# jianzongwu/betrayed-by-captions

Hardware: AMD Instinct MI355X
Metric: images/sec (COCO-shaped 1024x1024, 100 queries, forward-only) (higher is better)
Workload: dtype f32; 1 GPU; configs[1]: R50 + 100 queries, 1024x1024, batch 2/GPU, forward-only; global_batch=2, parallelism=replicas x1, precision=fp32 (parity mode, f16x3 MFMA), hip_graph=True, x3_overflow=False, library_fallbacks=0

## Files before the change

betrayed-by-captions_amd/_lib.py:

```python
import ctypes
import os

import torch

_HERE = os.path.dirname(os.path.abspath(__file__))
LIB_PATH = os.path.join(_HERE, 'lib', 'libcgg_hip.so')

CGG_F32 = 0
CGG_BF16 = 1

_c_int = ctypes.c_int
_c_vp = ctypes.c_void_p
_c_f = ctypes.c_float
_c_i64 = ctypes.c_int64

PROTOTYPES = {
    'cgg_version': (_c_int, []),
    'cgg_init': (_c_int, [_c_int]),
    'cgg_msda_forward_fused_vld': (_c_int, [_c_vp, _c_int, _c_vp, _c_vp, _c_vp, _c_int, _c_vp, _c_vp] + [_c_int] * 7 + [_c_vp]),
    'cgg_msda_backward_hostlevels_ws': (_c_int, [_c_vp, _c_int] + [_c_vp] * 8 + [_c_int] * 8 + [_c_vp, _c_i64, _c_vp, _c_vp]),
    'cgg_msda_backward_workspace_bytes': (_c_i64, [_c_vp, _c_vp] + [_c_int] * 7),
    'cgg_msda_read_levels': (_c_int, [_c_vp, _c_vp, _c_int, _c_int, _c_vp, _c_vp, _c_vp]),
    'cgg_last_error_string': (ctypes.c_char_p, []),
    'cgg_msda_forward': (_c_int, [_c_vp] * 6 + [_c_int] * 8 + [_c_vp]),
# ... 7 lines not shown
    'cgg_mask_logits': (_c_int, [_c_vp] * 5 + [_c_int] * 4 + [_c_vp]),
    'cgg_mask_logits_bits_astat': (_c_int, [_c_vp] * 3 + [_c_int] * 4 + [_c_vp]),
    'cgg_mask_logits_f32': (_c_int, [_c_vp] * 4 + [_c_int] * 4 + [_c_vp]),
    'cgg_mask_logits_backward_workspace_bytes': (_c_i64, [_c_int] * 4),
    'cgg_mask_logits_backward': (_c_int, [_c_vp] * 6 + [_c_int] * 5 + [_c_vp]),
    'cgg_attn_mask_fix_full_rows': (_c_int, [_c_vp, _c_int, _c_int, _c_vp]),
    'cgg_attn_mask_from_logits': (_c_int, [_c_vp, _c_vp] + [_c_int] * 5 + [_c_vp]),
    'cgg_masked_xattn_workspace_bytes': (_c_i64, [_c_int] * 5),
    'cgg_masked_xattn_forward': (_c_int, [_c_vp] * 5 + [_c_int] * 5 + [_c_f, _c_int, _c_vp]),
    'cgg_masked_xattn_forward_strided': (_c_int, [_c_vp, _c_vp, _c_int, _c_i64, _c_vp, _c_vp, _c_vp] + [_c_int] * 5 + [_c_f, _c_vp]),
    'cgg_masked_xattn_forward_x3': (_c_int, [_c_vp, _c_vp, _c_int, _c_i64, _c_vp, _c_vp, _c_vp] + [_c_int] * 5 + [_c_f, _c_vp]),
    'cgg_masked_xattn_forward_lse': (_c_int, [_c_vp] * 6 + [_c_int] * 5 + [_c_f, _c_int, _c_vp]),
    'cgg_masked_xattn_backward_workspace_bytes': (_c_i64, [_c_int] * 5),
    'cgg_masked_xattn_backward': (_c_int, [_c_vp] * 9 + [_c_int] * 5 + [_c_f, _c_int, _c_vp]),
    'cgg_masked_xattn_backward_x3': (_c_int, [_c_vp] * 10 + [_c_int] * 5 + [_c_f, _c_vp]),
    'cgg_window_attn_forward': (_c_int, [_c_vp] * 4 + [_c_int] * 7 + [_c_f, _c_vp]),
    'cgg_window_attn_backward_workspace_bytes': (_c_i64, [_c_int] * 5),
    'cgg_window_attn_backward': (_c_int, [_c_vp] * 7 + [_c_int] * 7 + [_c_f, _c_vp]),
    'cgg_grounding_pair_costs': (_c_int, [_c_vp] * 4 + [_c_int] * 5 + [_c_f, _c_vp]),
    'cgg_grounding_pair_costs_backward': (_c_int, [_c_vp] * 5 + [_c_int] * 5 + [_c_f, _c_vp]),
    'cgg_ce_rows_forward': (_c_int, [_c_vp] * 4 + [_c_int, _c_int, _c_i64, _c_i64, _c_int, _c_vp]),
    'cgg_ce_rows_backward': (_c_int, [_c_vp] * 4 + [_c_int, _c_int, _c_i64, _c_i64, _c_int, _c_vp]),
    'cgg_match_cost_rows': (_c_int, [_c_vp] * 4 + [_c_int, _c_int, _c_int, _c_vp]),
    'cgg_rle_encode_bitmasks': (_c_i64, [_c_vp, _c_int, _c_int, _c_int, _c_i64, _c_int, _c_int, _c_vp, _c_i64, _c_vp]),
    'cgg_masked_xattn_forward_bf16': (_c_int, [_c_vp] * 6 + [_c_int] * 5 + [_c_f, _c_int, _c_i64, _c_int, _c_vp]),
    'cgg_linear_rows': (_c_int, [_c_vp, _c_int, _c_vp, _c_vp, _c_vp, _c_int, _c_vp] + [_c_int] * 6 + [_c_vp]),
    'cgg_add_layernorm': (_c_int, [_c_vp] * 5 + [_c_int, _c_int, _c_f, _c_vp]),
    'cgg_linear_rows_packed_bytes': (_c_i64, [_c_int, _c_int]),
    'cgg_linear_rows_pack': (_c_int, [_c_vp, _c_vp, _c_int, _c_int, _c_vp]),
    'cgg_linear_rows_bf16': (_c_int, [_c_vp, _c_int, _c_vp, _c_vp, _c_vp, _c_int, _c_vp, _c_int, _c_vp, _c_vp, _c_f,
                                      _c_vp, _c_int, _c_vp, _c_int] + [_c_int] * 5 +
                             [_c_vp, _c_int, _c_int, _c_vp, _c_int, _c_int, _c_vp]),
    'cgg_decoder_tail_bf16': (_c_int, [_c_vp, _c_int, _c_i64, _c_int, _c_vp, _c_vp, _c_f, _c_vp, _c_int, _c_vp, _c_vp, _c_f] +
                              [_c_vp] * 12 + [_c_int, _c_int, _c_vp]),
    'cgg_self_attn_rows_bf16': (_c_int, [_c_vp, _c_int, _c_vp, _c_int, _c_vp] + [_c_int] * 4 + [_c_f, _c_vp]),
    'cgg_decoder_mid_bf16': (_c_int, [_c_vp, _c_int, _c_vp, _c_vp, _c_vp, _c_int, _c_vp, _c_vp, _c_f, _c_vp, _c_int] +
                             [_c_vp] * 5 + [_c_int, _c_int, _c_vp]),
    'cgg_decoder_ffn_bf16': (_c_int, [_c_vp, _c_int] + [_c_vp] * 5 + [_c_int] * 3 + [_c_vp]),
    'cgg_x3_packed_bytes': (_c_i64, [_c_int, _c_int]),
    'cgg_x3_pack': (_c_int, [_c_vp, _c_vp, _c_int, _c_int, _c_vp]),
    'cgg_linear_rows_x3': (_c_int, [_c_vp, _c_int, _c_vp, _c_vp, _c_vp, _c_int, _c_vp, _c_int, _c_vp, _c_vp, _c_f,
                                    _c_vp, _c_int, _c_vp, _c_int] + [_c_int] * 5 +
                           [_c_vp, _c_int, _c_int, _c_vp, _c_int, _c_int, _c_vp]),
    'cgg_decoder_tail_x3': (_c_int, [_c_vp, _c_int, _c_i64, _c_int, _c_vp, _c_vp, _c_f, _c_vp, _c_int, _c_vp, _c_vp, _c_f] +
                            [_c_vp] * 12 + [_c_int, _c_int, _c_vp]),
    'cgg_decoder_mid_x3': (_c_int, [_c_vp, _c_int, _c_vp, _c_vp, _c_vp, _c_int, _c_vp, _c_vp, _c_f, _c_vp, _c_int] +
                           [_c_vp] * 5 + [_c_int, _c_int, _c_vp]),
    'cgg_decoder_ffn_x3': (_c_int, [_c_vp, _c_int] + [_c_vp] * 5 + [_c_int] * 3 + [_c_vp]),
    'cgg_encoder_layer_tail_x3': (_c_int, [_c_vp] * 6 + [_c_f] + [_c_vp] * 6 + [_c_f, _c_vp, _c_int, _c_vp, _c_vp] +
                                  [_c_int] * 3 + [_c_vp]),
    'cgg_gemm_x3': (_c_int, [_c_vp, _c_int, _c_vp, _c_vp, _c_vp, _c_int, _c_vp, _c_int] + [_c_int] * 4 + [_c_vp]),
    'cgg_stem_conv7x7_x3_nchw': (_c_int, [_c_vp] * 4 + [_c_int] * 3 + [_c_vp]),
    'cgg_bias_relu_maxpool_nhwc_f32': (_c_int, [_c_vp] * 3 + [_c_int] * 4 + [_c_vp]),
    'cgg_gemm_x3_ex': (_c_int, [_c_vp, _c_int, _c_vp, _c_vp, _c_vp, _c_int, _c_int, _c_vp, _c_int, _c_vp, _c_int, _c_int] +
                       [_c_int] * 4 + [_c_vp]),
    'cgg_conv_x3_nhwc': (_c_int, [_c_vp] * 5 + [_c_int] * 10 + [_c_vp]),
    'cgg_gemm_x3s': (_c_int, [_c_vp, _c_int, _c_vp, _c_vp, _c_vp, _c_int, _c_int, _c_int, _c_vp, _c_int, _c_int] + [_c_int] * 4 + [_c_vp]),
    'cgg_gemm_x3s_batched': (_c_int, [_c_vp, _c_int, _c_int, _c_i64, _c_vp, _c_vp, _c_vp, _c_int, _c_int, _c_int, _c_vp, _c_int, _c_int] + [_c_int] * 4 + [_c_vp]),
    'cgg_conv_x3s_nhwc': (_c_int, [_c_vp] * 4 + [_c_int, _c_vp, _c_int] + [_c_int] * 10 + [_c_vp]),
    'cgg_x3a_encode': (_c_int, [_c_vp, _c_vp, _c_i64, _c_vp]),
    'cgg_x3a_decode': (_c_int, [_c_vp, _c_vp, _c_i64, _c_vp]),
    'cgg_x3_overflow_check': (_c_int, [_c_int, _c_vp, _c_vp]),
    'cgg_gemm_x3s_cfg': (_c_int, [_c_vp, _c_int, _c_vp, _c_vp, _c_vp, _c_int, _c_int, _c_int, _c_vp, _c_int, _c_int] + [_c_int] * 5 + [_c_vp]),
    'cgg_conv_x3s_nhwc_cfg': (_c_int, [_c_vp] * 4 + [_c_int, _c_vp, _c_int] + [_c_int] * 11 + [_c_vp]),
    'cgg_bias_relu_maxpool_nhwc_f32_x3a': (_c_int, [_c_vp] * 3 + [_c_int] * 4 + [_c_vp]),
    'cgg_group_norm_nhwc_f32_x3a': (_c_int, [_c_vp] * 4 + [_c_int] * 4 + [_c_f, _c_int, _c_vp, _c_int, _c_int, _c_i64, _c_int, _c_vp,
                                             _c_i64, _c_vp, _c_vp, _c_vp]),
    'cgg_encoder_layer_tail_x3a': (_c_int, [_c_vp] * 6 + [_c_f] + [_c_vp] * 6 + [_c_f, _c_vp, _c_int, _c_vp, _c_vp] +
                                   [_c_int] * 3 + [_c_vp]),
    'cgg_group_norm_nhwc_f32_stats': (_c_int, [_c_vp, _c_vp] + [_c_int] * 4 + [_c_vp]),
    'cgg_mask_feature_head_x3': (_c_int, [_c_vp] * 4 + [_c_f, _c_int] + [_c_vp] * 5 + [_c_int, _c_vp] + [_c_int] * 5 + [_c_vp]),
    'cgg_mask_feature_head_x3_cfg': (_c_int, [_c_vp] * 4 + [_c_f, _c_int] + [_c_vp] * 5 + [_c_int, _c_vp] + [_c_int] * 6 + [_c_vp]),
    'cgg_image_prep_u8': (_c_int, [_c_vp, _c_i64, _c_i64, _c_vp, _c_int, _c_vp, _c_vp, _c_vp, _c_int, _c_int, _c_vp, _c_int, _c_int, _c_vp]),
    'cgg_wgrad_x3_workspace_bytes': (_c_i64, [_c_int] * 3),
    'cgg_wgrad_x3': (_c_int, [_c_vp, _c_int, _c_vp, _c_int, _c_vp, _c_vp] + [_c_int] * 3 + [_c_vp]),
    'cgg_wgrad_bias_x3': (_c_int, [_c_vp, _c_int, _c_vp, _c_int, _c_vp, _c_vp, _c_vp] + [_c_int] * 3 + [_c_vp]),
    'cgg_transpose_f32': (_c_int, [_c_vp, _c_vp, _c_int, _c_int, _c_int, _c_vp]),
    'cgg_nchw_to_nhwc_pad1_f32': (_c_int, [_c_vp, _c_vp] + [_c_int] * 4 + [_c_vp]),
    'cgg_topk_select': (_c_int, [_c_vp, _c_int, _c_int, _c_int, _c_int, _c_vp, _c_vp]),
    'cgg_absmax_f32': (_c_int, [_c_vp, _c_int, _c_int, _c_int, _c_vp, _c_vp]),
    'cgg_relu_bwd_absmax_f32': (_c_int, [_c_vp, _c_vp, _c_vp, ctypes.c_longlong, _c_vp, _c_vp]),
    'cgg_gemm_x3_bwd': (_c_int, [_c_vp, _c_int, _c_vp, _c_vp, _c_vp, _c_int, _c_vp, _c_int, _c_vp] + [_c_int] * 3 + [_c_vp]),
    'cgg_gemm_x3_scaled': (_c_int, [_c_vp, _c_int, _c_vp, _c_vp, _c_vp, _c_vp, _c_int, _c_vp, _c_int] + [_c_int] * 4 + [_c_vp]),
    'cgg_conv_x3_nhwc_scaled': (_c_int, [_c_vp] * 6 + [_c_int] * 10 + [_c_vp]),
    'cgg_wgrad_x3_scaled': (_c_int, [_c_vp, _c_int, _c_vp, _c_vp, _c_int, _c_vp, _c_vp, _c_vp] + [_c_int] * 3 + [_c_vp]),
    'cgg_layernorm_chain': (_c_int, [_c_vp, _c_int, _c_vp, _c_vp, _c_f, _c_vp, _c_int, _c_vp, _c_vp, _c_f, _c_vp, _c_vp,
                                     _c_vp, _c_int, _c_int, _c_int, _c_i64, _c_vp]),
    'cgg_msda_prologue': (_c_int, [_c_vp, _c_int, _c_vp, _c_vp, _c_vp, _c_vp] + [_c_int] * 5 + [_c_vp]),
    'cgg_msda_prologue_backward': (_c_int, [_c_vp, _c_vp, _c_vp, _c_int, _c_vp, _c_vp] + [_c_int] * 5 + [_c_vp]),
    'cgg_msda_forward_fused_bf16': (_c_int, [_c_vp] * 4 + [_c_int] + [_c_vp] * 2 + [_c_int] * 7 + [_c_vp]),
    'cgg_msda_forward_fused_bf16_hm': (_c_int, [_c_vp] * 4 + [_c_int] + [_c_vp] * 2 + [_c_int] * 7 + [_c_vp]),
    'cgg_decoder_kv_pack_k': (_c_int, [_c_vp, _c_vp, _c_int, _c_int, _c_vp]),
    'cgg_decoder_kv_proj_bf16': (_c_int, [_c_vp] * 7 + [_c_int] * 4 + [_c_vp]),
    'cgg_add_layernorm_backward_partials': (ctypes.c_int64, [_c_int]),
    'cgg_add_layernorm_backward': (_c_int, [_c_vp] * 5 + [_c_int, _c_vp, _c_f] + [_c_vp] * 3 + [_c_int, _c_int, _c_vp]),
    'cgg_add_layernorm_backward_amax': (_c_int, [_c_vp] * 5 + [_c_int, _c_vp, _c_f] + [_c_vp] * 4 + [_c_int, _c_int, _c_vp]),
    'cgg_bottleneck64_bf16': (_c_int, [_c_vp] * 8 + [_c_int] * 5 + [_c_vp]),
    'cgg_encoder_proj_pack': (_c_int, [_c_vp, _c_vp, _c_int, _c_int, _c_vp]),
    'cgg_encoder_proj_bf16': (_c_int, [_c_vp] * 3 + [_c_int] + [_c_vp] * 6 + [_c_int] * 5 + [_c_vp]),
    'cgg_encoder_ffn_ln_kv_bf16': (_c_int, [_c_vp] * 7 + [_c_f, _c_vp, _c_vp, _c_int, _c_vp, _c_int] + [_c_vp] * 3 +
                                   [_c_int] * 3 + [_c_vp]),
    'cgg_encoder_layer_tail_bf16': (_c_int, [_c_vp] * 6 + [_c_f] + [_c_vp] * 6 + [_c_f, _c_vp, _c_int, _c_vp, _c_vp, _c_int] +
                                    [_c_vp] * 3 + [_c_int] * 3 + [_c_vp]),
    'cgg_encoder_ffn_ln_bf16': (_c_int, [_c_vp] * 7 + [_c_f, _c_vp, _c_int] + [_c_vp] * 3 + [_c_int] * 3 + [_c_vp]),
    'cgg_add_layernorm_kv': (_c_int, [_c_vp, _c_int, _c_vp, _c_int] + [_c_vp] * 4 + [_c_int, _c_vp, _c_int] + [_c_vp] * 3 +
                             [_c_int, _c_int, _c_f, _c_vp]),
# ... 97 lines not shown
```

betrayed-by-captions_amd/backbones.py:

```python
import os

import torch
import torch.nn as nn

from . import ops, runtime
from .registry import BACKBONES

FROZEN_FOLDED = os.environ.get('CGG_FROZEN_FOLDED', '1') != '0'
X3_STEM = os.environ.get('CGG_X3_STEM', '1') != '0'


class Bottleneck(nn.Module):
    expansion = 4

    def __init__(self, inplanes, planes, stride=1, downsample=None, style='pytorch'):
        super().__init__()
        s1, s2 = (1, stride) if style == 'pytorch' else (stride, 1)
        self.conv1 = nn.Conv2d(inplanes, planes, 1, stride=s1, bias=False)
        self.bn1 = nn.BatchNorm2d(planes)
        self.conv2 = nn.Conv2d(planes, planes, 3, stride=s2, padding=1, bias=False)
        self.bn2 = nn.BatchNorm2d(planes)
        self.conv3 = nn.Conv2d(planes, planes * 4, 1, bias=False)
        self.bn3 = nn.BatchNorm2d(planes * 4)
        self.relu = nn.ReLU(inplace=True)
# ... 248 lines not shown
            if name == 'stem':
                return [fold(self.conv1, self.bn1, stem=True)]
            seq = []
            for blk in getattr(self, name):
                if blk.downsample is not None:
                    seq.append(fold(blk.downsample[0], blk.downsample[1]))
                seq.append(fold(blk.conv1, blk.bn1))
                seq.append(fold(blk.conv2, blk.bn2))
                if isinstance(blk, Bottleneck):
                    seq.append(fold(blk.conv3, blk.bn3))
            return seq

        cache = self.__dict__.setdefault('_fold_cache_x3', {})
        names = ['stem'] + list(self.res_layers if upto is None else self.res_layers[:upto])
        out = []
        for name in names:
            mods = [self.conv1, self.bn1] if name == 'stem' else [getattr(self, name)]
            tensors = [t for m in mods for t in list(m.parameters()) + list(m.buffers())]
            key = (sum(t._version for t in tensors), str(self.conv1.weight.device))
            hit = cache.get(name)
            if hit is None or hit[0] != key:
                with torch.no_grad():
                    hit = (key, stage_seq(name))
                cache[name] = hit
            out.extend(hit[1])
        return out

    def _x3_ok(self):
        def conv_ok(c):
            return (c.groups == 1 and tuple(c.dilation) == (1, 1) and c.kernel_size[0] == c.kernel_size[1]
                    and c.stride[0] == c.stride[1] and c.padding[0] == c.padding[1] and c.in_channels % 32 == 0 and c.bias is None
                    and c.out_channels % 8 == 0 and c.kernel_size[0] * c.kernel_size[1] <= 32)
        for name in self.res_layers:
            for blk in getattr(self, name):
                convs = [blk.conv1, blk.conv2] + ([blk.conv3] if isinstance(blk, Bottleneck) else [])
                if blk.downsample is not None:
                    if not (isinstance(blk.downsample[0], nn.Conv2d) and isinstance(blk.downsample[1], nn.BatchNorm2d)):
                        return False
                    convs.append(blk.downsample[0])
                if not all(conv_ok(c) for c in convs):
                    return False
        return self.conv1.bias is None

    def _forward_x3(self, x, upto=None):
        import torch.nn.functional as F
        x3a = runtime.x3a_enabled()
        seq = iter(self._folded_x3(upto))
        w, b = next(seq)
        mp, c1 = self.maxpool, self.conv1
        if ((mp.kernel_size, mp.stride, mp.padding, mp.dilation, mp.ceil_mode) == (3, 2, 1, 1, False) and x.dtype == torch.float32
                and x.is_contiguous() and tuple(c1.weight.shape) == (64, 3, 7, 7) and tuple(c1.stride) == (2, 2)
                and tuple(c1.padding) == (3, 3) and tuple(c1.dilation) == (1, 1) and X3_STEM):
            pk, sc = runtime.derived_cached('stem_packed_x3', (w,), lambda: ops.pack_stem_weight_x3(w))
            x = ops.bias_relu_maxpool_nhwc_f32(ops.stem_conv7x7_x3(x, pk, sc), b, x3a=x3a)
        else:
            x = F.conv2d(x.float(), w, b, stride=c1.stride, padding=c1.padding)
            x = mp(torch.relu_(x)).permute(0, 2, 3, 1).contiguous()
            if x3a:
                x = ops.x3a_encode(x)

        def conv(x, c, relu, res=None):
            wk, bias = next(seq)
            if x3a:
                return ops.conv_x3s_nhwc(x, wk, c.out_channels, c.kernel_size[0], c.stride[0], c.padding[0], bias, res=res, relu=relu)
            return ops.conv_x3_nhwc(x, wk, c.out_channels, c.kernel_size[0], c.stride[0], c.padding[0], bias, res=res, relu=relu)

        outs = []
        for i, name in enumerate(self.res_layers):
            if upto is not None and i >= upto:
                break
            for blk in getattr(self, name):
                identity = x if blk.downsample is None else conv(x, blk.downsample[0], False)
                y = conv(x, blk.conv1, True)
                if isinstance(blk, Bottleneck):
                    y = conv(y, blk.conv2, True)
                    x = conv(y, blk.conv3, True, identity)
                else:
                    x = conv(y, blk.conv2, True, identity)
            if i in self.out_indices:
                outs.append(x)
        if upto is not None:
            dec = (lambda t: ops.x3a_decode(t)) if x3a else (lambda t: t)
            return [dec(o) for o in outs], dec(x)
        if x3a and self.x3a_outputs:
            return tuple(ops.as_x3a(o.permute(0, 3, 1, 2)) for o in outs)
        if x3a:
            return tuple(ops.x3a_decode(o).permute(0, 3, 1, 2) for o in outs)
        return tuple(o.permute(0, 3, 1, 2) for o in outs)

    def forward(self, x):
        frozen_bn = all(not m.training for m in self.modules() if isinstance(m, nn.BatchNorm2d))
        if runtime.is_bf16() and not torch.is_grad_enabled() and frozen_bn and x.is_cuda:
            return self._forward_folded(x)
        if runtime.x3_enabled() and not torch.is_grad_enabled() and frozen_bn and x.is_cuda:
            if self._x3_ok():
                return self._forward_x3(x)
            runtime.note_fallback('ResNet', 'a convolution outside the implicit-GEMM rules (groups, dilation, C % 32, N % 8): MIOpen f32')
        outs = []
        frozen_nhwc = []
        first = 0
        xn = None
        if (FROZEN_FOLDED and runtime.x3_enabled() and torch.is_grad_enabled() and frozen_bn and x.is_cuda and self.frozen_stages >= 1
                and not x.requires_grad and self._x3_ok() and x.dtype == torch.float32
                and not any(p.requires_grad for n in self.res_layers[:self.frozen_stages] for p in getattr(self, n).parameters())
                and not any(p.requires_grad for p in list(self.conv1.parameters()) + list(self.bn1.parameters()))):
            with torch.no_grad():
                fouts, xf = self._forward_x3(x, upto=self.frozen_stages)
# ... 49 lines not shown
```

betrayed-by-captions_amd/ops.py:

```python
import ctypes
import os
import math

import torch

from . import _lib
from ._lib import CGG_BF16, CGG_F32, CggError, check, dev_ptr, stream_ptr

_WS_CACHE = {}

KERNEL_EVENTS = None


KERNEL_META = None


class _timed:
    def __init__(self, name, **meta):
        self.name = name
        self.meta = meta
        self.on = KERNEL_EVENTS is not None and not torch.cuda.is_current_stream_capturing()

    def __enter__(self):
        if self.on:
# ... 2038 lines not shown

def pack_stem_weight(w):
    if tuple(w.shape) != (64, 3, 7, 7):
        raise CggError(f'pack_stem_weight: expected (64, 3, 7, 7), got {tuple(w.shape)}')
    wk = torch.zeros((64, 7, 8, 3), dtype=torch.float32, device=w.device)
    wk[:, :, :7, :] = w.detach().float().permute(0, 2, 3, 1)
    wk = torch.cat([wk.reshape(64, 168), torch.zeros((64, 8), dtype=torch.float32, device=w.device)], 1)
    frag = wk.view(2, 32, 11, 2, 8).permute(0, 2, 3, 1, 4).contiguous().to(torch.bfloat16)
    out = frag.view(torch.uint8).reshape(-1)
    assert out.numel() == _lib_().cgg_stem_conv7x7_packed_bytes()
    return out


def stem_conv7x7(img, packed):
    B, C, H, W = img.shape
    if C != 3 or img.dtype != torch.float32 or not img.is_contiguous():
        raise CggError('stem_conv7x7: img must be a contiguous (B, 3, H, W) float32 tensor')
    Ho, Wo = (H - 1) // 2 + 1, (W - 1) // 2 + 1
    y = torch.empty((B, Ho, Wo, 64), dtype=torch.bfloat16, device=img.device)
    check(_lib_().cgg_stem_conv7x7_nchw(dev_ptr(img), dev_ptr(packed), dev_ptr(y), B, H, W, stream_ptr(img.device)),
          'cgg_stem_conv7x7_nchw')
    return y


def pack_stem_weight_x3(w):
    if tuple(w.shape) != (64, 3, 7, 7):
        raise CggError(f'pack_stem_weight_x3: expected (64, 3, 7, 7), got {tuple(w.shape)}')
    wk = torch.zeros((64, 7, 8, 3), dtype=torch.float32, device=w.device)
    wk[:, :, :7, :] = w.detach().float().permute(0, 2, 3, 1)
    wk = torch.cat([wk.reshape(64, 168), torch.zeros((64, 8), dtype=torch.float32, device=w.device)], 1)
    amax = wk.abs().amax(1).clamp_min(1e-30)
    e = torch.floor(torch.log2(amax)) + 1
    s = torch.pow(2.0, 11 - e)
    ws = wk * s[:, None]
    hi = ws.to(torch.float16)
    lo = (ws - hi.float()).to(torch.float16)
    frag = lambda t: t.view(2, 32, 11, 2, 8).permute(0, 2, 3, 1, 4).contiguous().view(torch.uint8).reshape(-1)
    packed = torch.cat([frag(hi), frag(lo)])
    assert packed.numel() == 2 * _lib_().cgg_stem_conv7x7_packed_bytes()
    return packed, (1.0 / (s * 16.0)).float().contiguous()


def stem_conv7x7_x3(img, packed, wscale):
    B, C, H, W = img.shape
    if C != 3 or img.dtype != torch.float32 or not img.is_contiguous():
        raise CggError('stem_conv7x7_x3: img must be a contiguous (B, 3, H, W) float32 tensor')
    Ho, Wo = (H - 1) // 2 + 1, (W - 1) // 2 + 1
    y = torch.empty((B, Ho, Wo, 64), dtype=torch.float32, device=img.device)
    check(_lib_().cgg_stem_conv7x7_x3_nchw(dev_ptr(img), dev_ptr(packed), dev_ptr(wscale, 'wscale', torch.float32), dev_ptr(y), B, H, W,
                                           stream_ptr(img.device)), 'cgg_stem_conv7x7_x3_nchw')
    return y


def bias_relu_maxpool_nhwc_f32(x, bias, x3a=False):
    B, H, W, C = x.shape
    Ho, Wo = (H - 1) // 2 + 1, (W - 1) // 2 + 1
    y = torch.empty((B, Ho, Wo, C), dtype=torch.float32, device=x.device)
    fn = _lib_().cgg_bias_relu_maxpool_nhwc_f32_x3a if x3a else _lib_().cgg_bias_relu_maxpool_nhwc_f32
    rc = fn(dev_ptr(x, 'x', torch.float32), dev_ptr(bias, 'bias', torch.float32), dev_ptr(y), B, H, W, C, stream_ptr(x.device))
    check(rc, 'cgg_bias_relu_maxpool_nhwc_f32')
    return y


def linear_sum_assignment_batch(costs):
    if not costs:
        return []
    flat = torch.cat([c.detach().to(device='cpu', dtype=torch.float32).contiguous().reshape(-1) for c in costs]) \
        if len(costs) > 1 else costs[0].detach().to(device='cpu', dtype=torch.float32).contiguous().reshape(-1)
    nr = [int(c.shape[0]) for c in costs]
    nc = [int(c.shape[1]) for c in costs]
    sizes = [min(a, b) for a, b in zip(nr, nc)]
    total = sum(sizes)
    rows = torch.empty((max(total, 1),), dtype=torch.int64)
    cols = torch.empty((max(total, 1),), dtype=torch.int64)
    rc = _lib_().cgg_linear_sum_assignment_f32(ctypes.c_void_p(flat.data_ptr()) if flat.numel() else None, len(costs),
                                               _int_array(nr), _int_array(nc), ctypes.c_void_p(rows.data_ptr()),
                                               ctypes.c_void_p(cols.data_ptr()))
    check(rc, 'cgg_linear_sum_assignment_f32')
    out, o = [], 0
    for n in sizes:
        out.append((rows[o:o + n], cols[o:o + n]))
        o += n
    return out


def point_sample_planes(planes, index, points):
    N, H, W = planes.shape
    rows, P, _ = points.shape
    out = torch.empty((rows, P), dtype=torch.float32, device=planes.device)
    if rows == 0:
        return out
    check(_lib_().cgg_point_sample_planes(dev_ptr(planes, 'planes', torch.float32), dev_ptr(index, 'index', torch.int32),
                                          dev_ptr(points.contiguous(), 'points', torch.float32), dev_ptr(out), N, H, W, rows, P,
                                          stream_ptr(planes.device)), 'cgg_point_sample_planes')
    return out


class _PointSampleRowsFn(torch.autograd.Function):

    @staticmethod
    def forward(ctx, planes, points):
        planes = planes.contiguous()
        points = points.contiguous()
        rows, H, W = planes.shape
        idx = torch.arange(rows, dtype=torch.int32, device=planes.device)
        ctx.save_for_backward(points)
# ... 141 lines not shown
```

include/cgg_hip.h:

```cpp
#ifndef CGG_HIP_H_
#define CGG_HIP_H_

#include <stdint.h>

#ifdef __cplusplus
extern "C" {
#endif

#define CGG_VERSION 100

#define CGG_OK 0
#define CGG_EINVAL (-1)
#define CGG_EUNSUPPORTED (-2)
#define CGG_EALIGN (-3)
#define CGG_ELIBRARY (-4)

#define CGG_F32 0
#define CGG_BF16 1
#define CGG_F32_BF16MFMA 2
#define CGG_F32_X3 3

typedef void* cgg_stream_t;

int cgg_version(void);
// ... 146 lines not shown
                        float* y, float* yp, float* z, int rows, int N, int nsum, int64_t plane,
                        cgg_stream_t stream);

int cgg_decoder_tail_bf16(const float* planes, int nsum, int64_t plane_stride, int ld, const float* gamma_a,
                          const float* beta_a, float eps_a, const float* pos, int pos_rows, const float* gamma_b,
                          const float* beta_b, float eps_b, const void* w1, const float* b1, const void* w2,
                          const float* b2, const void* w3, const float* b3, const void* wq, const float* bq, float* y,
                          float* yp, float* mask_embed, float* qn, int M, int C, cgg_stream_t stream);

int cgg_decoder_mid_bf16(const float* core, int ldc, const void* wo, const float* bo, const float* res, int ldr,
                         const float* gamma, const float* beta, float eps, const float* pos, int pos_rows,
                         const void* wqkv, const float* bqkv, float* x1, float* q, float* kv, int M, int C,
                         cgg_stream_t stream);

int cgg_decoder_ffn_bf16(const float* x, int ldx, const void* w1, const float* b1, const void* w2, const float* b2,
                         float* planes, int M, int C, int F, cgg_stream_t stream);

int64_t cgg_x3_packed_bytes(int N, int K);
int cgg_x3_pack(const float* w, void* packed, int N, int K, cgg_stream_t stream);
int cgg_linear_rows_x3(const float* x, int ldx, const void* w_x3, const float* bias, const float* res,
                       int ldr, float* y, int ldy, const float* ln_gamma, const float* ln_beta, float ln_eps,
                       const float* pos, int pos_rows, float* yp, int ldyp, int M, int N, int K, int relu_cols,
                       int ksplit, const float* x2, int ldx2, int x2_col, float* y2, int ldy2, int y2_col,
                       cgg_stream_t stream);
int cgg_decoder_tail_x3(const float* planes, int nsum, int64_t plane_stride, int ld, const float* gamma_a,
                        const float* beta_a, float eps_a, const float* pos, int pos_rows, const float* gamma_b,
                        const float* beta_b, float eps_b, const void* w1, const float* b1, const void* w2,
                        const float* b2, const void* w3, const float* b3, const void* wq, const float* bq, float* y,
                        float* yp, float* mask_embed, float* qn, int M, int C, cgg_stream_t stream);
int cgg_decoder_mid_x3(const float* core, int ldc, const void* wo, const float* bo, const float* res, int ldr,
                       const float* gamma, const float* beta, float eps, const float* pos, int pos_rows,
                       const void* wqkv, const float* bqkv, float* x1, float* q, float* kv, int M, int C,
                       cgg_stream_t stream);
int cgg_decoder_ffn_x3(const float* x, int ldx, const void* w1, const float* b1, const void* w2, const float* b2,
                       float* planes, int M, int C, int F, cgg_stream_t stream);

int cgg_group_norm_nhwc_f32(const float* x, const float* gamma, const float* beta, void* ws, int B, int HW, int C, int groups,
                            float eps, int relu, const float* up_src, int up_h, int up_w, int64_t up_bstride, int W,
                            float* y32, int64_t y32_bstride, void* y16, const float* pos, void* yp16, int64_t y16_bstride,
                            cgg_stream_t stream);
int cgg_pack_mask_feature_nhwc_f32_x3(const float* feat, void* const* hi_host, void* const* lo_host, const int* pools_host,
                                      int n, int B, int C, int H, int W, cgg_stream_t stream);
int cgg_point_sample_nhwc_x3(const float* feat, const float* pts, void* hi, void* lo, int B, int H, int W, int C, int P_total,
                             int P_group, cgg_stream_t stream);
int cgg_encoder_layer_tail_x3(const float* a32, const float* x32, const void* wo_x3, const float* bo, const float* gamma0,
                              const float* beta0, float eps0, const void* w1_x3, const float* b1, const void* w2_x3,
                              const float* b2, const float* gamma1, const float* beta1, float eps1, const float* pos,
                              int pos_rows, float* y32, float* yp32, int M, int C, int F, cgg_stream_t stream);
int cgg_gemm_x3(const float* a, int lda, const void* w_x3, const float* bias, const float* res, int ldr, float* out, int ldc,
                int M, int N, int K, int relu, cgg_stream_t stream);
int cgg_stem_conv7x7_x3_nchw(const float* img, const void* w_packed, const float* wscale, float* out, int B, int H, int W,
                             cgg_stream_t stream);
int cgg_bias_relu_maxpool_nhwc_f32(const float* x, const float* bias, float* y, int B, int H, int W, int C, cgg_stream_t stream);
int cgg_gemm_x3_ex(const float* a, int lda, const void* w_x3, const float* bias, const float* res, int ldr, int res_mod, float* out,
                   int ldc, float* out2, int ldc2, int col2, int M, int N, int K, int relu, cgg_stream_t stream);
int cgg_conv_x3_nhwc(const float* x, const void* w_x3, const float* bias, const float* res, float* out, int B, int H, int W,
                     int C, int N, int KH, int KW, int stride, int pad, int relu, cgg_stream_t stream);

int cgg_gemm_x3s(const void* a_x3a, int lda, const void* w_x3, const float* bias, const void* res, int ldr, int res_fmt,
                 int res_mod, void* out, int ldc, int out_fmt, int M, int N, int K, int relu, cgg_stream_t stream);
int cgg_gemm_x3s_batched(const void* a_x3a, int lda, int rows_per_image, int64_t a_bstride, const void* w_x3, const float* bias,
                         const void* res, int ldr, int res_fmt, int res_mod, void* out, int ldc, int out_fmt, int M, int N, int K,
                         int relu, cgg_stream_t stream);
int cgg_conv_x3s_nhwc(const void* x_x3a, const void* w_x3, const float* bias, const void* res, int res_fmt, void* out,
                      int out_fmt, int B, int H, int W, int C, int N, int KH, int KW, int stride, int pad, int relu,
                      cgg_stream_t stream);
int cgg_x3a_encode(const float* x, void* out_x3a, int64_t n, cgg_stream_t stream);
int cgg_x3a_decode(const void* x_x3a, float* out, int64_t n, cgg_stream_t stream);
int cgg_x3_overflow_check(int reset, int* value_host, cgg_stream_t stream);
int cgg_gemm_x3s_cfg(const void* a_x3a, int lda, const void* w_x3, const float* bias, const void* res, int ldr, int res_fmt,
                     int res_mod, void* out, int ldc, int out_fmt, int M, int N, int K, int relu, int cfg, cgg_stream_t stream);
int cgg_conv_x3s_nhwc_cfg(const void* x_x3a, const void* w_x3, const float* bias, const void* res, int res_fmt, void* out,
                          int out_fmt, int B, int H, int W, int C, int N, int KH, int KW, int stride, int pad, int relu, int cfg,
                          cgg_stream_t stream);
int cgg_bias_relu_maxpool_nhwc_f32_x3a(const float* x, const float* bias, void* y_x3a, int B, int H, int W, int C,
                                       cgg_stream_t stream);
int cgg_group_norm_nhwc_f32_x3a(const float* x, const float* gamma, const float* beta, void* ws, int B, int HW, int C, int groups,
                                float eps, int relu, const void* up_src_x3a, int up_h, int up_w, int64_t up_bstride, int W,
                                void* y_x3a, int64_t y_bstride, const float* pos, void* yp_x3a, cgg_stream_t stream);

int64_t cgg_group_norm_nhwc_backward_workspace_bytes(int B, int HW, int groups);
int cgg_group_norm_nhwc_f32_backward(const float* x, const float* y, const float* dy, const float* stats, const float* gamma, void* ws,
                                     int B, int HW, int C, int groups, float eps, int relu, float* dx, float* tot, float* dlo, int lo_h,
                                     int lo_w, int W, int dx_padded, cgg_stream_t stream);
int cgg_group_norm_nhwc_f32_padout(const float* x, const float* gamma, const float* beta, void* ws, int B, int HW, int C, int groups,
                                   float eps, int relu, const float* up_src, int up_h, int up_w, int64_t up_bstride, int W,
                                   float* y_padded, cgg_stream_t stream);
int cgg_encoder_layer_tail_x3a(const float* a32, const void* x_x3a, const void* wo_x3, const float* bo, const float* gamma0,
                               const float* beta0, float eps0, const void* w1_x3, const float* b1, const void* w2_x3,
                               const float* b2, const float* gamma1, const float* beta1, float eps1, const float* pos,
                               int pos_rows, void* y_x3a, void* yp_x3a, int M, int C, int F, cgg_stream_t stream);
int cgg_group_norm_nhwc_f32_stats(const float* x, void* ws, int B, int HW, int C, int groups, cgg_stream_t stream);
int cgg_mask_feature_head_x3(const float* z, const void* gn_ws, const float* gamma, const float* beta, float eps, int groups,
                             const void* w_x3, const float* bias, void* const* hi_host, void* const* lo_host, const int* pools_host,
                             int n, float* mf, int B, int H, int W, int C, int N, cgg_stream_t stream);
int cgg_mask_feature_head_x3_cfg(const float* z, const void* gn_ws, const float* gamma, const float* beta, float eps, int groups,
                                 const void* w_x3, const float* bias, void* const* hi_host, void* const* lo_host,
                                 const int* pools_host, int n, float* mf, int B, int H, int W, int C, int N, int cfg,
                                 cgg_stream_t stream);

#define CGG_IMAGE_PREP_MAX_DIM 65535
int cgg_image_prep_u8(const uint8_t* staged, int64_t staged_bytes, int64_t table_offset, const int32_t* table_host, int B,
                      const float* mean, const float* std, const float* pad_val, int to_rgb, int pad_before_norm, float* out, int Hb,
                      int Wb, cgg_stream_t stream);

int cgg_transpose_f32(const float* in, float* out, int B, int R, int C, cgg_stream_t stream);
// ... 138 lines not shown
```

Before: 396.6 images/sec.

## Fuse stem 7x7 conv with bias, ReLU and maxpool into one kernel

Adds a HIP kernel that computes the 7x7 stride-2 stem convolution with split-precision MFMA on a tile covering a 4x16 pooled output region, stages the conv results in LDS, then applies the 3x3 stride-2 maxpool, bias and ReLU, and writes the pooled NHWC output (optionally in x3a encoding with an overflow flag). This avoids writing the full-resolution conv map to global memory and reading it back in a second kernel. In exchange it recomputes the conv at pooled-tile halo borders and adds LDS pressure. The old two-kernel path stays as a fallback.

```diff
diff --git a/betrayed-by-captions_amd/_lib.py b/betrayed-by-captions_amd/_lib.py
--- a/betrayed-by-captions_amd/_lib.py
+++ b/betrayed-by-captions_amd/_lib.py
@@ -83,6 +83,7 @@
     'cgg_gemm_x3': (_c_int, [_c_vp, _c_int, _c_vp, _c_vp, _c_vp, _c_int, _c_vp, _c_int] + [_c_int] * 4 + [_c_vp]),
     'cgg_stem_conv7x7_x3_nchw': (_c_int, [_c_vp] * 4 + [_c_int] * 3 + [_c_vp]),
     'cgg_bias_relu_maxpool_nhwc_f32': (_c_int, [_c_vp] * 3 + [_c_int] * 4 + [_c_vp]),
+    'cgg_stem_pool_x3': (_c_int, [_c_vp] * 5 + [_c_int] * 4 + [_c_vp]),
     'cgg_gemm_x3_ex': (_c_int, [_c_vp, _c_int, _c_vp, _c_vp, _c_vp, _c_int, _c_int, _c_vp, _c_int, _c_vp, _c_int, _c_int] +
                        [_c_int] * 4 + [_c_vp]),
     'cgg_conv_x3_nhwc': (_c_int, [_c_vp] * 5 + [_c_int] * 10 + [_c_vp]),
diff --git a/betrayed-by-captions_amd/backbones.py b/betrayed-by-captions_amd/backbones.py
--- a/betrayed-by-captions_amd/backbones.py
+++ b/betrayed-by-captions_amd/backbones.py
@@ -324,7 +324,10 @@
                 and x.is_contiguous() and tuple(c1.weight.shape) == (64, 3, 7, 7) and tuple(c1.stride) == (2, 2)
                 and tuple(c1.padding) == (3, 3) and tuple(c1.dilation) == (1, 1) and X3_STEM):
             pk, sc = runtime.derived_cached('stem_packed_x3', (w,), lambda: ops.pack_stem_weight_x3(w))
-            x = ops.bias_relu_maxpool_nhwc_f32(ops.stem_conv7x7_x3(x, pk, sc), b, x3a=x3a)
+            if ops.stem_pool_x3_ok(x, pk, sc, b, x3a):
+                x = ops.stem_pool_x3(x, pk, sc, b, x3a=x3a)
+            else:
+                x = ops.bias_relu_maxpool_nhwc_f32(ops.stem_conv7x7_x3(x, pk, sc), b, x3a=x3a)
         else:
             x = F.conv2d(x.float(), w, b, stride=c1.stride, padding=c1.padding)
             x = mp(torch.relu_(x)).permute(0, 2, 3, 1).contiguous()
diff --git a/betrayed-by-captions_amd/csrc/stem_pool.hip b/betrayed-by-captions_amd/csrc/stem_pool.hip
--- /dev/null
+++ b/betrayed-by-captions_amd/csrc/stem_pool.hip
@@ -0,0 +1,192 @@
+#include "x3.h"
+
+typedef __attribute__((ext_vector_type(4))) uint32_t u32x4;
+
+#define SP_PH 4
+#define SP_PW 16
+#define SP_CH (2 * SP_PH + 1)
+#define SP_CW (2 * SP_PW + 1)
+#define SP_NPIX (SP_CH * SP_CW)
+#define SP_NT 10
+#define SP_THREADS (32 * SP_NT)
+#define SP_IH (2 * SP_CH + 5)
+#define SP_IWP 72
+#define SP_KS 11
+#define SP_OS 36
+
+__global__ __launch_bounds__(SP_THREADS) void cgg_stem_pool_x3_kernel(const float* __restrict__ img, const u32x4* __restrict__ wp,
+                                                                      const float* __restrict__ wscale, const float* __restrict__ bias,
+                                                                      float* __restrict__ out, int H, int W, int Ho, int Wo, int Hp,
+                                                                      int Wp, int x3a, int* __restrict__ flag) {
+  constexpr int WFRAG = 2 * SP_KS * 64;
+  constexpr int TILE_EL = SP_IH * SP_IWP * 3;
+  constexpr int LDS_MAIN = 2 * (WFRAG * 16 + TILE_EL * 2), LDS_STAGE = SP_NPIX * SP_OS * 4;
+  constexpr int LDS_BYTES = LDS_MAIN > LDS_STAGE ? LDS_MAIN : LDS_STAGE;
+  static_assert(LDS_BYTES <= 65536, "static LDS");
+  __shared__ __attribute__((aligned(16))) unsigned char lds_raw[LDS_BYTES];
+  u32x4* wl = reinterpret_cast<u32x4*>(lds_raw);
+  uint16_t* tile = reinterpret_cast<uint16_t*>(lds_raw + 2 * WFRAG * 16);
+  float* ob = reinterpret_cast<float*>(lds_raw);
+  const int tid = threadIdx.x, lane = tid & 63, wave = tid >> 6;
+  const int j = lane & 31, hi = lane >> 5;
+  const int b = blockIdx.z, py0 = blockIdx.y * SP_PH, px0 = blockIdx.x * SP_PW;
+  const int cy0 = 2 * py0 - 1, cx0 = 2 * px0 - 1;
+  const int iy0 = 2 * cy0 - 3, ix0 = 2 * cx0 - 3;
+
+  constexpr int WIT = (2 * WFRAG + SP_THREADS - 1) / SP_THREADS;
+  u32x4 wv[WIT];
+#pragma unroll
+  for (int it = 0; it < WIT; ++it) {
+    const int i = tid + SP_THREADS * it;
+    wv[it] = i < 2 * WFRAG ? wp[i] : u32x4{0u, 0u, 0u, 0u};
+  }
+
+  const float* ib = img + (size_t)b * 3 * H * W;
+  constexpr int NIT = (TILE_EL + SP_THREADS - 1) / SP_THREADS;
+  float tv[NIT];
+#pragma unroll
+  for (int it = 0; it < NIT; ++it) {
+    const int i = tid + SP_THREADS * it;
+    const int c = i / (SP_IH * SP_IWP);
+    const int rem = i - c * (SP_IH * SP_IWP);
+    const int r = rem / SP_IWP, col = rem - r * SP_IWP;
+    const int iy = iy0 + r, ix = ix0 + col;
+    tv[it] = 0.f;
+    if (i < TILE_EL && iy >= 0 && iy < H && ix >= 0 && ix < W) tv[it] = ib[((size_t)c * H + iy) * W + ix];
+  }
+#pragma unroll
+  for (int it = 0; it < NIT; ++it) {
+    const int i = tid + SP_THREADS * it;
+    const int c = i / (SP_IH * SP_IWP);
+    const int rem = i - c * (SP_IH * SP_IWP);
+    if (i < TILE_EL) {
+      uint16_t h, l;
+      cgg_x3_split1(tv[it], h, l);
+      tile[rem * 3 + c] = h;
+      tile[TILE_EL + rem * 3 + c] = l;
+    }
+  }
+#pragma unroll
+  for (int it = 0; it < WIT; ++it) {
+    const int i = tid + SP_THREADS * it;
+    if (i < 2 * WFRAG) wl[i] = wv[it];
+  }
+  __syncthreads();
+
+  int poff[2];
+#pragma unroll
+  for (int nt = 0; nt < 2; ++nt) {
+    int p = (2 * wave + nt) * 32 + j;
+    p = p < SP_NPIX ? p : SP_NPIX - 1;
+    const int r = p / SP_CW, c = p - r * SP_CW;
+    poff[nt] = (2 * r * SP_IWP + 2 * c) * 3;
+  }
+  f32x16 acc[2][2];
+#pragma unroll
+  for (int nt = 0; nt < 2; ++nt)
+#pragma unroll
+    for (int mt = 0; mt < 2; ++mt)
+#pragma unroll
+      for (int r = 0; r < 16; ++r) acc[nt][mt][r] = 0.f;
+#pragma unroll
+  for (int ks = 0; ks < SP_KS; ++ks) {
+    const int g = 2 * ks + hi;
+    const int ky = g / 3, part = g - 3 * ky;
+    const int koff = (ky > 6 ? 6 : ky) * SP_IWP * 3 + 8 * part;
+#pragma unroll
+    for (int nt = 0; nt < 2; ++nt) {
+      const uint16_t* src = tile + poff[nt] + koff;
+      const uint32_t* s32 = reinterpret_cast<const uint32_t*>(src);
+      const u32x4 bv = {s32[0], s32[1], s32[2], s32[3]};
+      const uint32_t* l32 = reinterpret_cast<const uint32_t*>(src + TILE_EL);
+      const u32x4 bl = {l32[0], l32[1], l32[2], l32[3]};
+#pragma unroll
+      for (int mt = 0; mt < 2; ++mt)
+        cgg_x3_mfma(acc[nt][mt], wl[(mt * SP_KS + ks) * 64 + lane], wl[WFRAG + (mt * SP_KS + ks) * 64 + lane], bv, bl);
+    }
+  }
+
+  const int pxl = (tid >> 2) & (SP_PW - 1), pyl = tid >> 6, grp = tid & 3;
+  const int py = py0 + pyl, px = px0 + pxl;
+  const bool mine = tid < SP_PH * SP_PW * 4 && py < Hp && px < Wp;
+#pragma unroll
+  for (int mt = 0; mt < 2; ++mt) {
+    __syncthreads();
+#pragma unroll
+    for (int nt = 0; nt < 2; ++nt) {
+      const int p = (2 * wave + nt) * 32 + j;
+      if (p < SP_NPIX) {
+#pragma unroll
+        for (int gq = 0; gq < 4; ++gq) {
+          const int ch = 8 * gq + 4 * hi;
+          const f32x4 sc = *reinterpret_cast<const f32x4*>(wscale + 32 * mt + ch);
+          *reinterpret_cast<f32x4*>(ob + p * SP_OS + ch) =
+              f32x4{acc[nt][mt][4 * gq] * sc[0], acc[nt][mt][4 * gq + 1] * sc[1], acc[nt][mt][4 * gq + 2] * sc[2],
+                    acc[nt][mt][4 * gq + 3] * sc[3]};
+        }
+      }
+    }
+    __syncthreads();
+    if (mine) {
+      const float ninf = -__builtin_inff();
+      f32x4 m0 = {ninf, ninf, ninf, ninf}, m1 = m0;
+#pragma unroll
+      for (int dy = 0; dy < 3; ++dy) {
+        const int r = 2 * pyl + dy;
+        if (cy0 + r < 0 || cy0 + r >= Ho) continue;
+#pragma unroll
+        for (int dx = 0; dx < 3; ++dx) {
+          const int c = 2 * pxl + dx;
+          if (cx0 + c < 0 || cx0 + c >= Wo) continue;
+          const float* s = ob + (r * SP_CW + c) * SP_OS + 8 * grp;
+          const f32x4 v0 = *reinterpret_cast<const f32x4*>(s), v1 = *reinterpret_cast<const f32x4*>(s + 4);
+#pragma unroll
+          for (int k = 0; k < 4; ++k) {
+            m0[k] = fmaxf(m0[k], v0[k]);
+            m1[k] = fmaxf(m1[k], v1[k]);
+          }
+        }
+      }
+      const int ch = 32 * mt + 8 * grp;
+      const f32x4 b0 = *reinterpret_cast<const f32x4*>(bias + ch), b1 = *reinterpret_cast<const f32x4*>(bias + ch + 4);
+      f32x4 o0, o1;
+#pragma unroll
+      for (int k = 0; k < 4; ++k) {
+        o0[k] = fmaxf(m0[k] + b0[k], 0.f);
+        o1[k] = fmaxf(m1[k] + b1[k], 0.f);
+      }
+      float* dst = out + ((((size_t)b * Hp + py) * Wp + px) * 64 + ch);
+      if (!x3a) {
+        *reinterpret_cast<f32x4*>(dst) = o0;
+        *reinterpret_cast<f32x4*>(dst + 4) = o1;
+      } else {
+        uint2 h0, l0, h1, l1;
+        cgg_x3_split4(o0, h0, l0);
+        cgg_x3_split4(o1, h1, l1);
+        *reinterpret_cast<u32x4*>(dst) = u32x4{h0.x, h0.y, h1.x, h1.y};
+        *reinterpret_cast<u32x4*>(dst + 4) = u32x4{l0.x, l0.y, l1.x, l1.y};
+        const bool ok0 = fmaxf(fmaxf(o0[0], o0[1]), fmaxf(o0[2], o0[3])) * CGG_X3_ASCALE <= CGG_X3A_MAX;
+        const bool ok1 = fmaxf(fmaxf(o1[0], o1[1]), fmaxf(o1[2], o1[3])) * CGG_X3_ASCALE <= CGG_X3A_MAX;
+        if (flag && !(ok0 && ok1)) atomicOr(flag, 1);
+      }
+    }
+  }
+}
+
+int* cgg_x3_overflow_flag_ptr();
+
+extern "C" int cgg_stem_pool_x3(const float* img, const void* w_packed, const float* wscale, const float* bias, void* out, int B, int H,
+                                int W, int x3a, cgg_stream_t stream) {
+  CGG_REQUIRE(img && w_packed && wscale && bias && out, CGG_EINVAL, "cgg_stem_pool_x3: null pointer");
+  CGG_REQUIRE(B > 0 && H > 0 && W > 0 && B <= 65535, CGG_EINVAL, "cgg_stem_pool_x3: bad sizes");
+  CGG_REQUIRE(cgg_aligned16(img) && cgg_aligned16(w_packed) && cgg_aligned16(wscale) && cgg_aligned16(bias) && cgg_aligned16(out),
+              CGG_EALIGN, "cgg_stem_pool_x3: pointers must be 16-byte aligned");
+  const int Ho = (H - 1) / 2 + 1, Wo = (W - 1) / 2 + 1;
+  const int Hp = (Ho - 1) / 2 + 1, Wp = (Wo - 1) / 2 + 1;
+  CGG_REQUIRE((Hp + SP_PH - 1) / SP_PH <= 65535, CGG_EUNSUPPORTED, "cgg_stem_pool_x3: H=%d too large", H);
+  int* flag = x3a ? cgg_x3_overflow_flag_ptr() : nullptr;
+  hipLaunchKernelGGL(cgg_stem_pool_x3_kernel, dim3((Wp + SP_PW - 1) / SP_PW, (Hp + SP_PH - 1) / SP_PH, B), dim3(SP_THREADS), 0,
+                     (hipStream_t)stream, img, (const u32x4*)w_packed, wscale, bias, (float*)out, H, W, Ho, Wo, Hp, Wp, x3a, flag);
+  CGG_CHECK_LAUNCH("cgg_stem_pool_x3");
+  return CGG_OK;
+}
diff --git a/betrayed-by-captions_amd/ops.py b/betrayed-by-captions_amd/ops.py
--- a/betrayed-by-captions_amd/ops.py
+++ b/betrayed-by-captions_amd/ops.py
@@ -2114,6 +2114,47 @@
     return y
 
 
+def _stem_pool_x3_why(img, packed, wscale, bias, x3a=False):
+    ts = (img, packed, wscale, bias)
+    if not all(isinstance(t, torch.Tensor) for t in ts):
+        return 'tensor operands expected'
+    if img.dim() != 4 or img.shape[1] != 3 or img.dtype != torch.float32 or not img.is_contiguous():
+        return 'img must be a contiguous (B, 3, H, W) float32 tensor'
+    if not all(t.is_cuda for t in ts):
+        return 'operands must live on a ROCm device'
+    if min(img.shape) < 1 or img.shape[0] > 65535:
+        return f'empty image or batch > 65535 {tuple(img.shape)}'
+    if (wscale.dtype != torch.float32 or bias.dtype != torch.float32 or wscale.numel() != 64 or bias.numel() != 64
+            or not wscale.is_contiguous() or not bias.is_contiguous() or packed.dtype != torch.uint8 or not packed.is_contiguous()):
+        return 'packed (uint8), wscale (64,) and bias (64,) float32, contiguous, expected'
+    if any(t.data_ptr() % 16 for t in ts):
+        return 'pointers must be 16-byte aligned'
+    return None
+
+
+def stem_pool_x3_ok(img, packed, wscale, bias, x3a=False):
+    try:
+        return _stem_pool_x3_why(img, packed, wscale, bias, x3a) is None
+    except Exception:
+        return False
+
+
+def stem_pool_x3(img, packed, wscale, bias, x3a=False):
+    why = _stem_pool_x3_why(img, packed, wscale, bias, x3a)
+    if why is not None:
+        raise CggError(f'stem_pool_x3: {why}')
+    B, _, H, W = img.shape
+    Ho, Wo = (H - 1) // 2 + 1, (W - 1) // 2 + 1
+    Hp, Wp = (Ho - 1) // 2 + 1, (Wo - 1) // 2 + 1
+    if len(packed.view(-1)) != 2 * _lib_().cgg_stem_conv7x7_packed_bytes():
+        raise CggError('stem_pool_x3: packed is not a pack_stem_weight_x3 image')
+    y = torch.empty((B, Hp, Wp, 64), dtype=torch.float32, device=img.device)
+    rc = _lib_().cgg_stem_pool_x3(dev_ptr(img), dev_ptr(packed), dev_ptr(wscale, 'wscale', torch.float32),
+                                  dev_ptr(bias, 'bias', torch.float32), dev_ptr(y), B, H, W, int(bool(x3a)), stream_ptr(img.device))
+    check(rc, 'cgg_stem_pool_x3')
+    return y
+
+
 def bias_relu_maxpool_nhwc_f32(x, bias, x3a=False):
     B, H, W, C = x.shape
     Ho, Wo = (H - 1) // 2 + 1, (W - 1) // 2 + 1
diff --git a/include/cgg_hip.h b/include/cgg_hip.h
--- a/include/cgg_hip.h
+++ b/include/cgg_hip.h
@@ -222,6 +222,8 @@
 int cgg_stem_conv7x7_x3_nchw(const float* img, const void* w_packed, const float* wscale, float* out, int B, int H, int W,
                              cgg_stream_t stream);
 int cgg_bias_relu_maxpool_nhwc_f32(const float* x, const float* bias, float* y, int B, int H, int W, int C, cgg_stream_t stream);
+int cgg_stem_pool_x3(const float* img, const void* w_packed, const float* wscale, const float* bias, void* out, int B, int H, int W,
+                     int x3a, cgg_stream_t stream);
 int cgg_gemm_x3_ex(const float* a, int lda, const void* w_x3, const float* bias, const float* res, int ldr, int res_mod, float* out,
                    int ldc, float* out2, int ldc2, int col2, int M, int N, int K, int relu, cgg_stream_t stream);
 int cgg_conv_x3_nhwc(const float* x, const void* w_x3, const float* bias, const float* res, float* out, int B, int H, int W,
diff --git a/scratch/stem_pool_bench.py b/scratch/stem_pool_bench.py
--- /dev/null
+++ b/scratch/stem_pool_bench.py
@@ -0,0 +1,89 @@
+import os
+import sys
+
+sys.path.insert(0, os.path.dirname(os.path.dirname(os.path.abspath(__file__))))
+import torch
+import cgg_amd
+from cgg_amd import ops
+
+dev = torch.device('cuda')
+N_LAUNCH, ROUNDS, COPIES = 20, 5, 4
+lines = []
+
+
+def say(s):
+    print(s, flush=True)
+    lines.append(s)
+
+
+def graph_of(fn):
+    s = torch.cuda.Stream()
+    s.wait_stream(torch.cuda.current_stream())
+    with torch.cuda.stream(s):
+        for i in range(3):
+            fn(i)
+    torch.cuda.current_stream().wait_stream(s)
+    torch.cuda.synchronize()
+    g = torch.cuda.CUDAGraph()
+    with torch.cuda.graph(g):
+        keep = [fn(i) for i in range(N_LAUNCH)]
+    g.replay()
+    torch.cuda.synchronize()
+    return g, keep
+
+
+def time_replay(g):
+    s, e = torch.cuda.Event(enable_timing=True), torch.cuda.Event(enable_timing=True)
+    torch.cuda.synchronize()
+    s.record()
+    g.replay()
+    e.record()
+    torch.cuda.synchronize()
+    return s.elapsed_time(e) / N_LAUNCH * 1e3
+
+
+def run(B, H, W):
+    g = torch.Generator().manual_seed(H)
+    imgs = [(torch.randn(B, 3, H, W, generator=g) * 2).to(dev) for _ in range(COPIES)]
+    w = (torch.randn(64, 3, 7, 7, generator=g) / 12).to(dev)
+    b = torch.randn(64, generator=g).to(dev)
+    pk, sc = ops.pack_stem_weight_x3(w)
+
+    def two(i):
+        return ops.bias_relu_maxpool_nhwc_f32(ops.stem_conv7x7_x3(imgs[i % COPIES], pk, sc), b, x3a=True)
+
+    def conv(i):
+        return ops.stem_conv7x7_x3(imgs[i % COPIES], pk, sc)
+
+    def fused(i):
+        return ops.stem_pool_x3(imgs[i % COPIES], pk, sc, b, x3a=True)
+
+    same = torch.equal(two(1).view(torch.int32), fused(1).view(torch.int32))
+    fns = dict(two_calls=two, fused=fused, conv_only=conv)
+    graphs = {k: graph_of(f) for k, f in fns.items()}
+    t = {k: [] for k in fns}
+    for _ in range(ROUNDS):
+        for k in fns:
+            t[k].append(time_replay(graphs[k][0]))
+    med = {k: sorted(v)[len(v) // 2] for k, v in t.items()}
+    Ho, Wo = (H - 1) // 2 + 1, (W - 1) // 2 + 1
+    Hp, Wp = (Ho - 1) // 2 + 1, (Wo - 1) // 2 + 1
+    b_in, b_raw, b_out = B * 3 * H * W * 4, B * Ho * Wo * 64 * 4, B * Hp * Wp * 64 * 4
+    say(f'(B, 3, H, W) = ({B}, 3, {H}, {W}): conv map {Ho} x {Wo}, pooled {Hp} x {Wp}; outputs bit-identical: {same}')
+    for k in fns:
+        say(f'  {k:9s} median {med[k]:7.1f} us   runs ' + ' '.join(f'{x:.1f}' for x in t[k]))
+    say(f'  bytes moved: two calls {(b_in + 2 * b_raw + b_out) / 1e6:.1f} MB (image {b_in / 1e6:.1f} + raw map written and read '
+        f'2 x {b_raw / 1e6:.1f} + pooled {b_out / 1e6:.1f}), fused {(b_in + b_out) / 1e6:.1f} MB')
+    ok = max(t['fused']) < min(t['two_calls'])
+    say(f'  fused saves {med["two_calls"] - med["fused"]:.1f} us = {100 * (1 - med["fused"] / med["two_calls"]):.1f} %; slowest fused run '
+        f'{max(t["fused"]):.1f} vs fastest two-call run {min(t["two_calls"]):.1f}: {"PASS" if ok else "FAIL"}')
+    return same
+
+
+ok = True
+for shape in ((2, 1024, 1024), (2, 800, 1344)):
+    ok = run(*shape) and ok
+if len(sys.argv) > 1:
+    with open(sys.argv[1], 'w') as f:
+        f.write('\n'.join(lines) + '\n')
+sys.exit(0 if ok else 1)
```

After: 397.4 images/sec, median of 6. No clear change (+0.2%).
